# Nico59000/Ternary-image-codec

Measured on AMD Instinct MI355X. Metric: Mpix/s encode+decode 8K RS(26,20), higher is better.
Workload: dtype u8

## Files before the change

ternary-image-codec_amd/csrc/t3_api_decode.cpp:

```cpp
#include <hip/hip_runtime.h>
#include <math.h>
#include <stdio.h>
#include <string.h>

#include <stdlib.h>

#include <algorithm>
#include <mutex>
#include <vector>

#include "../../include/t3hip.h"
#include "t3_ctx.hpp"
#include "t3_dec_plan.hpp"
#include "t3_decode.h"
#include "t3_host.hpp"
#include "t3_repair.h"
#include "t3_window.h"

using namespace t3;

namespace {
struct HdrCheck { HdrExpect ex; uint32_t hs; uint32_t* verdict; const uint8_t* in; };

int launch_hdr_compare(const HdrCheck* h, hipStream_t s) {
    if (!h) return T3_OK;
    hipLaunchKernelGGL(hdr_compare_kernel, dim3(1), dim3(128), 0, s, h->in, h->ex, h->hs, h->verdict);
    HIPCHK(hipGetLastError());
    return T3_OK;
}
template <class A> int settle_header(A& a, const HdrCheck* h, bool whole_frame, hipStream_t s) {
    static const bool no_fold = getenv("T3HIP_HDR_KERNEL") != nullptr;
    if (!h || !a.tile_ctr || !whole_frame || no_fold || h->hs > 96u || ((uintptr_t)h->in & 3u) != 0) return launch_hdr_compare(h, s);
    a.verdict = h->verdict; a.hdr_in = h->in; a.hdr_n = h->hs; memcpy(a.hx, h->ex.b, 96);
    a.fail = a.tile_ctr + 64u * a.n_classes + 16u;
    return T3_OK;
}


int ensure_fx_tables(DecodeTables& tab, int k) {
    const int ki = k_index(k);
    if (!tab.synd_lut[ki]) {
        std::vector<uint32_t> img; build_syndrome_lut(k, img);
        HIPCHK(hipMalloc((void**)&tab.synd_lut[ki], img.size() * 4u));
        HIPCHK(hipMemcpy(tab.synd_lut[ki], img.data(), img.size() * 4u, hipMemcpyHostToDevice));
    }
    if (!tab.roots[ki]) {
        const Field& F = field(); const int t = (26 - k) / 2;
        size_t n = 1; for (int i = 0; i < t; ++i) n *= 27;
        std::vector<uint32_t> tbl(n);
        for (size_t idx = 0; idx < n; ++idx) {
            uint8_t sg[5] = {1, 0, 0, 0, 0}; { size_t v = idx; for (int q = 1; q <= t; ++q) { sg[q] = (uint8_t)(v % 27); v /= 27; } }
            uint32_t mask = 0;
            for (int i = 0; i < 26; ++i) {
                const uint8_t x = F.t.exp[i == 0 ? 0 : 26 - i];
                uint8_t acc = sg[t];
                for (int q = t - 1; q >= 0; --q) acc = F.t.add[F.t.mul[acc * 27 + x] * 27 + sg[q]];
                if (acc == 0) mask |= 1u << i;
            }
            tbl[idx] = mask;
        }
        HIPCHK(hipMalloc((void**)&tab.roots[ki], n * 4));
        HIPCHK(hipMemcpy(tab.roots[ki], tbl.data(), n * 4, hipMemcpyHostToDevice));
    }
    if (!tab.synd_afrag[ki]) {
        std::vector<uint32_t> af; build_mfma_syndrome(k, af);
        HIPCHK(hipMalloc((void**)&tab.synd_afrag[ki], af.size() * 4)); HIPCHK(hipMemcpy(tab.synd_afrag[ki], af.data(), af.size() * 4, hipMemcpyHostToDevice));
    }
    if (!tab.synd_T) {
        std::vector<uint32_t> img; build_syndrome_T(img);
        HIPCHK(hipMalloc((void**)&tab.synd_T, img.size() * 4)); HIPCHK(hipMemcpy(tab.synd_T, img.data(), img.size() * 4, hipMemcpyHostToDevice));
        build_syndrome_T(img, 16);
        HIPCHK(hipMalloc((void**)&tab.synd_T16, img.size() * 4)); HIPCHK(hipMemcpy(tab.synd_T16, img.data(), img.size() * 4, hipMemcpyHostToDevice));
        uint8_t sm[kFx2SmallBytes + kFx2ModBytes]; build_fx2_small(sm); build_fx2_mod(sm + kFx2SmallBytes);
        HIPCHK(hipMalloc((void**)&tab.fx2_small, sizeof sm)); HIPCHK(hipMemcpy(tab.fx2_small, sm, sizeof sm, hipMemcpyHostToDevice));
    }
    if (!tab.fma) {
        const Field& F = field();
        std::vector<uint8_t> t(kFmaBytes, 0);
        for (int x = 0; x < 27; ++x) for (int y = 0; y < 27; ++y) for (int c = 0; c < 27; ++c) t[(size_t)(x * 27 + y) * 27 + c] = F.t.add[c * 27 + F.t.mul[x * 27 + y]];
        HIPCHK(hipMalloc((void**)&tab.fma, t.size())); HIPCHK(hipMemcpy(tab.fma, t.data(), t.size(), hipMemcpyHostToDevice));
    }
    return T3_OK;
}

int rgb_dequant_tables(Ctx& c, const uint8_t** out) {
    uint8_t*& d = c.rgb.dequant;
    if (!d) {
        uint8_t t[328]; memset(t, 0, sizeof t);
        auto cl = [](long v) { return v < 0 ? 0 : (v > 255 ? 255 : v); };
        for (int q = 0; q <= 242; ++q) t[q] = (uint8_t)cl(lround(q * (255.0 / 242.0)));
        for (int q = -40; q <= 40; ++q) t[244 + q + 40] = (uint8_t)cl(lround(128 + q * (128.0 / 40.0)));
        HIPCHK(hipMalloc((void**)&d, sizeof t)); HIPCHK(hipMemcpy(d, t, sizeof t, hipMemcpyHostToDevice));
    }
    *out = d; return T3_OK;
}

template <class A, class F> int bind_groups(Ctx& c, A& a, F attach) {
    std::lock_guard<std::mutex> lk(c.tab_mu);
    for (uint32_t g = 0; g < a.n_grp; ++g) { const int k = 26 - (int)a.grp[g].r; const int rc = ensure_fx_tables(c.dec, k); if (rc) return rc; attach(a.grp[g], k_index(k)); }
    a.fma = c.dec.fma; return T3_OK;
}
int bind_uep(UepPlan& p, void* d_out, uint32_t* d_fail) {
    Ctx& c = ctx(); DecUepArgs& a = p.a;
    { const int rc = bind_groups(c, a, [&](DecUepArgs::Grp& G, int ki) { G.afrag = c.dec.synd_afrag[ki]; G.roots = c.dec.roots[ki]; a.ttab = c.dec.synd_T16; a.small = c.dec.fx2_small; }); if (rc) return rc; }
    a.out = d_out; a.fail = d_fail;
    p.fn = by_r(p.ra, [&](auto A) { return by_r(p.rb, [&](auto B) -> const void* {
        if constexpr (decltype(A)::value >= decltype(B)::value) return (const void*)decode_uep_px_kernel<decltype(A)::value, decltype(B)::value>; else return nullptr; }); });
    if (!p.fn) return T3_E_ARG;
    return resident_grid(c, p.fn, 512, a.lds_bytes, a.n_tiles, true, &p.grid);
}
int bind_stream(StreamPlan& p, void* d_out, uint32_t* d_fail) {
    Ctx& c = ctx(); DecStArgs& a = p.a;
    { const int rc = bind_groups(c, a, [&](DecStArgs::Grp& G, int ki) { G.lut = c.dec.synd_lut[ki]; G.roots = c.dec.roots[ki]; a.tab = c.dec.fxtab; }); if (rc) return rc; }
    a.fail = d_fail; p.e.out = d_out;
    p.emit_fn = p.to_pixels ? (const void*)emit_stream_kernel<true> : (const void*)emit_stream_kernel<false>;
    { const int rc = resident_grid(c, (const void*)decode_stream_kernel, 512, a.lds_bytes, a.n_tiles, false, &p.grid); if (rc) return rc; }
    return resident_grid(c, p.emit_fn, 512, p.e.lds_bytes, p.e.n_steps, false, &p.emit_grid);
}

int launch_fixed_fused(FusedPlan& p, const uint8_t* body, const HdrCheck* hdr, hipStream_t s) {
    Ctx& c = ctx(); DecFx2Args& a = p.a; const uint32_t grid = p.grid;
    a.in = body;
#ifdef T3_DEC_STAMPS
    static uint64_t* d_dbg = nullptr; static int calls = 0;
    if (!d_dbg) HIPCHK(hipMalloc((void**)&d_dbg, 16 * 8 * 4096));
    HIPCHK(hipMemsetAsync(d_dbg, 0, 16 * 8 * 4096, s));
    a.dbg = d_dbg;
#endif
    if (p.tickets) tile_tickets(c, s, 1, grid, &a.tile_ctr, &a.n_classes);
    { const int rc = settle_header(a, hdr, p.whole_frame, s); if (rc) return rc; }
    void* args[] = {(void*)&a};
    HIPCHK(hipLaunchKernel(p.fn, dim3(grid), dim3(p.threads), args, a.lds_bytes, s));
#ifdef T3_DEC_STAMPS
    if (++calls == 8 && p.tickets) {
        std::vector<uint64_t> h(16 * grid);
        HIPCHK(hipStreamSynchronize(s));
        HIPCHK(hipMemcpy(h.data(), d_dbg, h.size() * 8, hipMemcpyDeviceToHost));
        double acc[16] = {0};
        for (uint32_t w = 0; w < grid; ++w) for (int i = 0; i < 16; ++i) acc[i] += (double)h[16 * w + i];
        fprintf(stderr, "[t3 dec stamps] grid=%u (%d per CU) tiles=%u lds=%u  mean cycles/WG: producer sets+e1=%.0f barrier=%.0f total=%.0f | consumer bm=%.0f rendezvous=%.0f d5=%.0f barrier=%.0f total=%.0f  clock=%.3f GHz  us/WG=%.1f\n",
                grid, (int)((grid + c.n_cu - 1) / c.n_cu), a.n_tiles, a.lds_bytes, acc[0] / grid, acc[1] / grid, acc[6] / grid, acc[8 + 2] / grid, acc[8 + 3] / grid, acc[8 + 4] / grid, acc[8 + 5] / grid, acc[8 + 6] / grid,
                acc[6] / acc[7] * 0.1, acc[7] / grid * 0.01);
        uint64_t s0 = ~0ull, s1 = 0, e1 = 0; int late = 0;
        for (uint32_t w = 0; w < grid; ++w) { s0 = std::min(s0, h[16 * w + 2]); s1 = std::max(s1, h[16 * w + 2]); e1 = std::max(e1, h[16 * w + 3]); }
        for (uint32_t w = 0; w < grid; ++w) if (h[16 * w + 2] - s0 > 1000) ++late;
        fprintf(stderr, "[t3 dec stamps]   prologue (kernel entry -> first tile's input landed, wave 0): mean %.0f cycles/WG\n", acc[4] / grid);
        fprintf(stderr, "[t3 dec stamps]   timeline (us from first loop start): last start=%.1f last end=%.1f  workgroups starting >10 us late=%d\n", (s1 - s0) * 0.01, (e1 - s0) * 0.01, late);
    }
#endif
    return T3_OK;
}

int launch_fixed_uep(UepPlan& p, const uint8_t* body, const HdrCheck* hdr, hipStream_t s) {
    Ctx& c = ctx(); DecUepArgs& a = p.a;
    void* d_e; int rc = scratch(c, Scratch::StreamWork, (size_t)a.n_sym + 64, &d_e, s); if (rc) return rc;
    a.in = body; a.edge = (uint8_t*)d_e;
    tile_tickets(c, s, 2, p.grid, &a.tile_ctr, &a.n_classes);
    rc = settle_header(a, hdr, true, s); if (rc) return rc;
    void* args[] = {(void*)&a};
    HIPCHK(hipLaunchKernel(p.fn, dim3(p.grid), dim3(512), args, a.lds_bytes, s));
    HIPCHK(hipLaunchKernel((const void*)uep_edge_kernel, dim3((3u * a.n_tiles + 1u + 255u) / 256u), dim3(256), args, 0, s));
    return T3_OK;
}

int launch_fixed_stream(StreamPlan& p, const uint8_t* body, const HdrCheck* hdr, hipStream_t s) {
    void* d_y; int rc = scratch(ctx(), Scratch::StreamWork, (size_t)p.a.n_sym + 64, &d_y, s); if (rc) return rc;
    p.a.in = body; p.a.ystream = (uint8_t*)d_y; p.e.ystream = (const uint8_t*)d_y;
    rc = launch_hdr_compare(hdr, s); if (rc) return rc;
    void* args[] = {(void*)&p.a}; void* eargs[] = {(void*)&p.e};
    HIPCHK(hipLaunchKernel((const void*)decode_stream_kernel, dim3(p.grid), dim3(512), args, p.a.lds_bytes, s));
    HIPCHK(hipLaunchKernel(p.emit_fn, dim3(p.emit_grid), dim3(512), eargs, p.e.lds_bytes, s));
    return T3_OK;
}

int decode_body(const void* d_in, uint64_t n_in, const t3_cfg& cfg, uint64_t n_raw, const uint8_t next[3],
                void* d_out, uint64_t cap_units, uint64_t* n_out, int to_pixels, uint32_t* d_fail, hipStream_t s, const HdrCheck* hdr) {
    const bool fixed = cfg.mode == T3_MODE_FIXED;
    const bool want_rgb = to_pixels == 2;
    if (((uintptr_t)d_in & 1u) != 0 || (to_pixels == 1 && ((uintptr_t)d_out & 1u) != 0)) return T3_E_ARG;
    if (want_rgb && !fixed) return 1;
    Ctx& c = ctx();
    DecArgs a; memset(&a, 0, sizeof a);
    EmitArgs e; memset(&e, 0, sizeof e);
    a.in = (const uint8_t*)d_in; a.fail = d_fail; a.tab = c.d_tab; a.fixed = fixed ? 1 : 0;
    const ScrCycle sc = scrambler_cycle_from_next(next, cfg.seed_s0);
    a.cyc24 = sc.cyc24; a.pre0 = sc.pre[0]; a.pre1 = sc.pre[1];
    a.beacon_on = (cfg.beacon_enabled && cfg.beacon_words_period > 0) ? 1 : 0; a.period = cfg.beacon_words_period; a.slot = cfg.beacon_band_slot;
    uint64_t use_syms, n_words, total = 0;
    if (!fixed) {
        DecLayoutCompat D; plan_decode_compat(n_in, cfg, D);
        a.hdr_syms = 54;
        for (int b = 0; b < 9; ++b) { a.band_k[b] = D.band_k[b]; a.band_blocks[b] = D.band_blocks[b]; a.band_first[b] = total; a.band_off[b] = D.use_off[b]; total += D.band_blocks[b]; }
        use_syms = D.use_syms; n_words = D.out_words;
    } else {
        t3_layout L; int rc = plan(n_raw, cfg, L); if (rc) return T3_E_HEADER;
        if (L.out_words > n_in) return T3_E_HEADER;
        a.hdr_syms = 90; a.n_sym = L.n_sym;
        for (int b = 0; b < 9; ++b) { a.band_k[b] = L.band_k[b]; a.band_blocks[b] = L.band_blocks[b]; a.band_first[b] = total; a.band_off[b] = L.band_body_off[b]; total += L.band_blocks[b]; }
        use_syms = L.n_sym; n_words = n_raw;
        const uint64_t funits = want_rgb ? cap_units : to_pixels ? 2 * n_words : n_words;
        if (want_rgb && (cap_units > 2 * n_words || cap_units + 1 < 2 * n_words || L.interleave2d)) return 1;
        if (want_rgb && !single_k(L)) return 1;
        if (funits <= cap_units && (!to_pixels || ((uintptr_t)d_out & 15u) == 0) && !generic_decode() && 9 * n_in < (1ull << 32)) {
            const bool bcn_ok = L.beacon_on && cfg.beacon_band_slot < 9 && cfg.beacon_words_period >= 2 && cfg.beacon_words_period < (1u << 27) && getenv("T3HIP_BEACON_PASS") == nullptr;
            const uint64_t bytes = L.beacon_on ? L.body_syms : 9 * n_in; const uint32_t hs = L.beacon_on ? 0u : L.header_syms;
            FusedPlan fp; UepPlan up; StreamPlan sp;
            const FusedForm form = (FusedForm)to_pixels;
            int path = 0, frc = bcn_ok ? plan_fixed_fused(9 * n_in, L.header_syms, L, sc, funits, form, fp, cfg.beacon_band_slot, cfg.beacon_words_period)
                                       : plan_fixed_fused(bytes, hs, L, sc, funits, form, fp);
            if (frc == 1 && want_rgb) return 1;
            if (frc == 1 && to_pixels == 1) { path = 1; frc = plan_fixed_uep(bytes, hs, cfg, L, sc, funits, getenv("T3HIP_TWO_KERNEL_DECODE") != nullptr, up); }
            static const uint32_t lut_bytes[4] = {synd_lut_bytes(24), synd_lut_bytes(22), synd_lut_bytes(20), synd_lut_bytes(18)};
            if (frc == 1) { path = 2; frc = plan_fixed_stream(bytes, hs, cfg, L, sc, funits, to_pixels, lut_bytes, sp); }
            if (frc == T3_OK) frc = path == 0 ? bind_fused(fp, d_out, d_fail) : path == 1 ? bind_uep(up, d_out, d_fail) : bind_stream(sp, d_out, d_fail);
            if (frc < 0) return frc;
            if (frc == T3_OK) {
                const uint8_t* body = (const uint8_t*)d_in;
                if (L.beacon_on && !(path == 0 && bcn_ok)) {
                    void* d_b; int brc = scratch(c, Scratch::StreamBody, L.body_syms + 64, &d_b, s); if (brc) return brc;
                    DebeaconArgs d; d.framed = (const uint8_t*)d_in + L.header_syms; d.framed_bytes = 9 * n_in - L.header_syms; d.body = (uint8_t*)d_b; d.body_syms = L.body_syms; d.period = cfg.beacon_words_period; d.slot = cfg.beacon_band_slot;
                    if (L.body_syms) { hipLaunchKernelGGL(debeacon_kernel, dim3(blocks_for((L.body_syms + 15) / 16, 1u << 20)), dim3(256), 0, s, d); HIPCHK(hipGetLastError()); }
                    body = (const uint8_t*)d_b;
                }
                frc = path == 0 ? launch_fixed_fused(fp, body, hdr, s) : path == 1 ? launch_fixed_uep(up, body, hdr, s) : launch_fixed_stream(sp, body, hdr, s);
                if (frc == T3_OK) *n_out = funits;
                return frc;
            }
        }
    }
    if (want_rgb) return 1;
    a.total_blocks = total;
    const uint64_t units = to_pixels ? 2 * n_words : n_words;
    *n_out = units;
    if (units > cap_units) return T3_E_CAPACITY;
    void* d_use; int rc = scratch(c, Scratch::StreamWork, use_syms + 64, &d_use, s); if (rc) return rc;
    rc = launch_hdr_compare(hdr, s); if (rc) return rc;
    a.use = (uint8_t*)d_use;
    if (total) { hipLaunchKernelGGL(dec_gather_rs_kernel, dim3(blocks_for(total, 1u << 20)), dim3(256), 0, s, a); HIPCHK(hipGetLastError()); }
    e.use = (const uint8_t*)d_use; e.use_syms = use_syms; e.out = d_out; e.n_words = n_words; e.to_pixels = to_pixels ? 1 : 0;
    const bool il = cfg.profile == T3_P5_RS26_22_2D && cfg.tile_w && cfg.tile_h && use_syms;
    e.il_on = il ? 1 : 0;
    if (il) fill_interleave(e, cfg, use_syms);
    if (n_words) { hipLaunchKernelGGL(dec_emit_kernel, dim3(blocks_for(n_words, 1u << 20)), dim3(256), 0, s, e); HIPCHK(hipGetLastError()); }
    return T3_OK;
}

int read_header(const void* d_in, uint64_t n_in, int mode, t3_cfg* seen, uint64_t* n_raw, uint8_t next[3], hipStream_t s) {
    const uint64_t hw = mode == T3_MODE_FIXED ? 10 : 6;
    if (n_in < hw) return T3_E_HEADER;
    Ctx& c = ctx();
    std::lock_guard<std::mutex> lk(c.mail_mu);
    uint8_t*& h = c.mail.header;
    if (!h) HIPCHK(hipHostMalloc((void**)&h, 128, hipHostMallocDefault));
    HIPCHK(hipMemcpyAsync(h, d_in, hw * 9, hipMemcpyDeviceToHost, s));
    HIPCHK(hipStreamSynchronize(s));
    uint8_t hb[96]; memcpy(hb, h, hw * 9);
    return header_parse(hb, n_in, mode, *seen, n_raw, next);
}

int fill_window_crop(WinCropArgs& a, const void* d_run, uint64_t first_px, uint64_t stream_px, uint32_t fw, uint32_t fh, uint32_t x0, uint32_t y0, uint32_t w, uint32_t h,
                     void* d_out, bool rgb) {
    Ctx& c = ctx();
    memset(&a, 0, sizeof a);
    if (rgb) { std::lock_guard<std::mutex> lk(c.tab_mu); const int rc = rgb_dequant_tables(c, &a.dq); if (rc) return rc; }
    a.run = (const uint8_t*)d_run; a.out = (uint8_t*)d_out; a.first_px = first_px; a.stream_px = stream_px;
    a.out_bytes = (uint64_t)w * h * (rgb ? 3u : 6u);
    a.lead = (uint32_t)((uintptr_t)d_out & 15u); a.n_gran = (a.lead + a.out_bytes + 15u) / 16u;
    a.fw = fw; a.fh = fh; a.x0 = x0; a.y0 = y0; a.w = w; a.h = h;
    a.wide = a.out_bytes >= (1ull << 31) ? 1u : 0u;
    if (!a.wide) a.div_row = to_dev(fastdiv(rgb ? w : 3u * w)); else a.div_row.d = rgb ? w : 3u * w;
    return a.n_gran > (1ull << 38) || 3ull * w >= (1ull << 32) ? T3_E_ARG : T3_OK;
}
int launch_window_crop(const void* d_run, uint64_t first_px, uint64_t stream_px, uint32_t fw, uint32_t fh, uint32_t x0, uint32_t y0, uint32_t w, uint32_t h,
                       void* d_out, int out_fmt, hipStream_t s) {
    WinCropArgs a; const bool rgb = out_fmt == 2;
    { const int rc = fill_window_crop(a, d_run, first_px, stream_px, fw, fh, x0, y0, w, h, d_out, rgb); if (rc) return rc; }
    const void* fn = rgb ? (const void*)window_crop_kernel<true> : (const void*)window_crop_kernel<false>;
    void* args[] = {(void*)&a};
    HIPCHK(hipLaunchKernel(fn, dim3((unsigned)((a.n_gran + 255u) / 256u)), dim3(256), args, 0, s));
    return T3_OK;
}
int launch_window_crop_frames(const void* d_run, uint64_t run_stride, uint64_t first_px, uint64_t stream_px, uint32_t fw, uint32_t fh, uint32_t x0, uint32_t y0,
                              uint32_t w, uint32_t h, void* d_out, uint64_t out_stride, int out_fmt, uint32_t n_frames, hipStream_t s) {
    WinCropFramesArgs fa; memset(&fa, 0, sizeof fa);
    const bool rgb = out_fmt == 2;
    { const int rc = fill_window_crop(fa.a, d_run, first_px, stream_px, fw, fh, x0, y0, w, h, d_out, rgb); if (rc) return rc; }
    fa.run_stride = run_stride; fa.out_stride = out_stride;
    if (n_frames > 65535u || (((uintptr_t)d_run | (uintptr_t)d_out | run_stride | out_stride) & 15u)) return T3_E_ARG;
    const void* fn = rgb ? (const void*)window_crop_frames_kernel<true> : (const void*)window_crop_frames_kernel<false>;
    void* args[] = {(void*)&fa};
    HIPCHK(hipLaunchKernel(fn, dim3((unsigned)((fa.a.n_gran + 255u) / 256u), n_frames), dim3(256), args, 0, s));
    return T3_OK;
}
// ... 415 lines not shown
```

ternary-image-codec_amd/csrc/t3_decode.h:

```cpp
#pragma once
#include <stdint.h>

#include "t3_device.h"
#include "t3_rs_core.h"

namespace t3 {

struct DecArgs {
    const uint8_t* in;
    uint8_t* use;
    uint32_t* fail;
    const RsTables* tab;
    uint32_t fixed;
    uint32_t hdr_syms;
    uint32_t band_k[9];
    uint64_t band_blocks[9];
    uint64_t band_first[9];
    uint64_t band_off[9];
    uint64_t total_blocks;
    uint64_t n_sym;
    uint32_t beacon_on, period, slot;
    uint32_t cyc24, pre0, pre1;
};

struct EmitArgs {
    const uint8_t* use; uint64_t use_syms;
    void* out; uint64_t n_words;
    uint32_t to_pixels;
    uint32_t il_on, il_w, il_A; DevDiv div_A, div_w;
};

struct FxTables {
    uint8_t mul[729], add[729], sub[729];
    uint8_t inv[27], neg[27], exp[26];
    uint8_t descr[3][32];
    uint8_t pad_[37];
};
static_assert(sizeof(FxTables) == 2400, "FxTables layout");
constexpr int kFxHdr = 512, kFxTab = kFxHdr, kFxLut = 3072;

constexpr int kFx2Cnt = 160, kFx2Sync = 168, kFx2Abort = 172, kFx2Next = 176, kFx2FailWg = 184, kFx2Small = 192;
#ifndef T3_DEC_PX_THREADS
#define T3_DEC_PX_THREADS 512
#endif
#ifndef T3_DEC_PX_AREG
#define T3_DEC_PX_AREG 2
#endif
#ifndef T3_DEC_PX_TCOP
#define T3_DEC_PX_TCOP 16
#endif
#ifndef T3_DEC_PX_NB
#define T3_DEC_PX_NB 52
#endif
#ifndef T3_DEC_QCAP
#define T3_DEC_QCAP 256
#endif
constexpr int kFx2ModSeq = 3072, kFx2TSeq = 3584, kFx2ModPx = 512, kFx2TPx = 1024, kFx2QCap = T3_DEC_QCAP;
constexpr uint32_t kEraQCap = 512;
static_assert(T3_DEC_PX_THREADS % 128 == 0 && T3_DEC_PX_THREADS <= 1024 && T3_DEC_PX_NB % 26 == 0 && 9 * T3_DEC_PX_NB <= T3_DEC_PX_THREADS && T3_DEC_PX_NB < 2048, "pixel-decoder geometry");
struct DecFx2Args {
    const uint8_t* in; uint64_t in_bytes;
    void* out; uint64_t n_units;
    uint32_t* fail;
    const uint32_t* ttab; const uint8_t* small; const uint32_t* afrag;
    const uint8_t* fma; uint32_t fma_off;
    const uint32_t* roots;
    uint32_t k, nb, n_tiles, TS;
    DevDiv div_nb;
    uint32_t n_sym;
    uint32_t hdr_syms;
    uint32_t band_blocks[9]; uint64_t band_body_off[9]; uint32_t band_boff6[9];
    uint32_t cyc24, pre0, pre1;
    uint32_t* tile_ctr; uint32_t n_classes;
    uint32_t* verdict; const uint8_t* hdr_in; uint32_t hdr_n; uint32_t hx[24];
    uint32_t pat[48], pat_off;
    uint32_t y_off, y_stride, q_off, q_stride, o_off, af_off, lds_bytes;
    uint32_t bcn_slot, bcn_pb; DevDiv bcn_div;
    const uint8_t* dq; uint32_t dq_off;
    uint64_t* dbg;
};

struct DecFramesArgs {
    DecFx2Args a;
    uint64_t in_stride, out_stride;
    uint32_t n_frames, n_total;
    DevDiv div_tiles;
};

struct DecEraWinArgs {
    DecFx2Args a;
    uint32_t fw; DevDiv div_fw;
    uint32_t x0, y0, w, rows_end;
    uint32_t first_px, n_px;
};
struct DecEraWinFramesArgs { DecEraWinArgs w; uint64_t in_stride, out_stride; uint32_t n_frames, n_total; DevDiv div_tiles; };

constexpr int kUepMaxGrp = 2;
struct DecUepArgs {
    const uint8_t* in; uint64_t in_bytes;
    void* out; uint64_t n_units;
    uint32_t* fail;
    const uint32_t* ttab; const uint8_t* small; const uint8_t* fma; uint32_t fma_off;
    struct Grp { uint32_t r, nb, n_items, af_off, q_rel, q_cap; DevDiv div_nb; const uint32_t* afrag; const uint32_t* roots; uint8_t bands[12]; } grp[kUepMaxGrp];
    uint32_t n_grp;
    uint32_t pair_tab[8];
    uint32_t TS, n_tiles, n_sym, hdr_syms;
    uint32_t band_blocks[9]; uint64_t band_body_off[9]; uint32_t band_boff6[9];
    uint32_t pat[48], pat_off, rec_off;
    uint32_t y_off, y_stride, q_off, q_stride, lds_bytes;
    uint32_t* tile_ctr; uint32_t n_classes;
    uint32_t* verdict; const uint8_t* hdr_in; uint32_t hdr_n; uint32_t hx[24];
    uint32_t il_on, il_w, il_A; DevDiv div_A, div_w;
    uint8_t* edge;
};

constexpr int kStMaxGrp = 4;
struct DecStArgs {
    const uint8_t* in; uint64_t in_bytes;
    uint8_t* ystream;
    uint32_t* fail;
    const FxTables* tab; const uint8_t* fma; uint32_t fma_off;
    struct Grp { uint32_t r, nb, n_items, wave0, n_waves, lut_off, lut_bytes; const uint32_t* lut; const uint32_t* roots; uint8_t bands[12]; } grp[kStMaxGrp];
    uint32_t n_grp, n_slots;
    uint32_t n_tiles, TS;
    uint32_t n_sym, hdr_syms;
    uint32_t band_blocks[9]; uint64_t band_body_off[9]; uint32_t band_boff6[9];
    uint32_t cyc24, pre0, pre1;
    uint32_t y_off, lds_bytes;
};
struct EmitStArgs {
    const uint8_t* ystream; uint32_t n_sym;
    void* out; uint64_t n_units;
    uint32_t span;
    uint32_t n_steps;
    uint32_t il_on, il_w, il_A, il_fast;
    DevDiv div_A, div_w;
    uint32_t sym_off, o_off, lds_bytes;
};
struct DescrArgs { uint8_t* words; uint64_t n_bytes; uint32_t cyc24, pre0, pre1; };
constexpr int kStageBlocks = 64, kStageThreads = 9 * 64, kStageRunBytes = 9 * 26 * kStageBlocks;
struct StageDecArgs {
    const uint8_t* body;
    uint8_t* out;
    uint64_t* n_valid;
    const RsTables* tab;
    uint32_t band_k[9], band_fixed[9];
    uint64_t band_off[9];
    uint64_t nb;
    uint32_t bcn_band;
    uint64_t bcn_blocks;
    DevDiv div_p1;
};
struct HdrExpect { uint8_t b[96]; };
struct DebeaconArgs { const uint8_t* framed; uint64_t framed_bytes; uint8_t* body; uint64_t body_syms; uint32_t period, slot; };

#if defined(__HIPCC__)
__global__ void dec_gather_rs_kernel(const DecArgs a);
template <int R, bool BCN> __global__ void decode_fixed_kernel(const DecFx2Args a);
template <int R, bool RGB, bool BCN> __global__ void decode_fixed_px_kernel(const DecFx2Args a);
template <int R, bool RGB, bool BCN> __global__ void decode_era_px_kernel(const DecFx2Args a);
__global__ void era_verdict_kernel(const uint32_t* rep6, uint32_t* verdict4);
template <int R, bool RGB, bool BCN> __global__ void decode_era_frames_px(const DecFramesArgs fa);
template <int R, bool RGB, bool BCN> __global__ void decode_era_window_px(const DecEraWinArgs wa);
template <int R, bool RGB, bool BCN> __global__ void decode_era_frames_window_px(const DecEraWinFramesArgs fa);
template <int R, bool RGB, bool BCN = false> __global__ void dec_frames_px(const DecFramesArgs fa);
__global__ void decode_stream_kernel(const DecStArgs a);
template <int RA, int RB> __global__ void decode_uep_px_kernel(const DecUepArgs a);
__global__ void uep_edge_kernel(const DecUepArgs a);
template <bool TO_PIXELS> __global__ void emit_stream_kernel(const EmitStArgs a);
__global__ void debeacon_kernel(const DebeaconArgs a);
__global__ void dec_emit_kernel(const EmitArgs a);
__global__ void descramble_words_kernel(const DescrArgs a);
__global__ void stage_decode_kernel(const StageDecArgs a);
__global__ void fill_u64_kernel(uint64_t* p, uint64_t v);
__global__ void rs_decode_blocks_kernel(uint8_t* code, uint64_t n_blocks, int k, int fixed, const RsTables* tab, uint8_t* data, uint8_t* ok);
__global__ void inject_errors_kernel(uint8_t* syms, uint64_t n_blocks, uint32_t seed, int max_err);
__global__ void hdr_compare_kernel(const uint8_t* in, HdrExpect expect, uint32_t n, uint32_t* mismatch);
#endif

}
```

ternary-image-codec_amd/csrc/t3_decode_px_body.inc:

```
    constexpr uint32_t TCOP = T3_DEC_PX_TCOP, TBASE = kFx2TPx, MT = kFx2ModPx, QCAP = kFx2QCap;
    constexpr uint32_t NW = T3_DEC_PX_THREADS / 128;
    const uint32_t tid = threadIdx.x, lane = tid & 63u, wave = __builtin_amdgcn_readfirstlane(tid >> 6);
#ifdef T3_DEC_STAMPS
    const uint64_t st_entry = __builtin_amdgcn_s_memtime(); uint64_t st_first = 0;
#endif
    const Tickets tk = tickets_setup(a);
    tk.first(tid);
    uint32_t* const failp = a.verdict ? (uint32_t*)(lds + kFx2FailWg) : a.fail;
    if (tid == 0) *(uint32_t*)(lds + kFx2FailWg) = 0u;
    stage_constants<TCOP, TBASE, MT>(a, tid, blockDim.x);
    if constexpr (RGB) { if (tid < 82u) *(uint32_t*)(lds + a.dq_off + 4u * tid) = ((const uint32_t*)a.dq)[tid]; }
    __syncthreads();
#ifdef T3_DEC_STAMPS
    uint64_t st_acc[6] = {0, 0, 0, 0, 0, 0}, st_prev = __builtin_amdgcn_s_memtime(), st_t0 = st_prev, st_rt0 = __builtin_amdgcn_s_memrealtime();
#endif
    if (a.verdict && px_header_wg(args) && wave == 2u * NW - 1u) {
        uint32_t want = 0;
#pragma unroll
        for (uint32_t q = 0; q < 24; ++q) want = lane == q ? a.hx[q] : want;
        px_header_check(args, want, lane);
    }
    const uint8_t* body = a.in + a.hdr_syms;
    const uint32_t n_items = 9u * a.nb;
    const uint32_t units_tile = (a.TS / 13u) * 3u;
    uint32_t cur = blockIdx.x, nxt = tk.next(1u);

    if (wave < NW) {
        const uint32_t n = lane & 31u, h = lane >> 5;
        Geo geo[2][2]; uint32_t off0[2][2];
        const uint32_t t_off = 26u * a.nb;
#pragma unroll
        for (uint32_t p = 0; p < 2; ++p) for (uint32_t q = 0; q < 2; ++q) geo[p][q] = fx2_geo<R>(wave * 128u + p * 64u + q * 32u + n, n_items, a.nb, a.div_nb, 0u, off0[p][q]);
        auto has = [&](uint32_t pass, uint32_t set, uint32_t tile) -> bool { Geo g = geo[pass][set]; asm volatile("" : "+v"(g)); return fx2_has_block<R>(g, tile, a.n_tiles, a.nb); };
        auto run_of = [&](uint32_t pass, uint32_t set, uint32_t tile, const uint8_t* fbody) -> Run<BCN> { return load_run<BCN>(a, fbody, has(pass, set, tile) ? off0[pass][set] + tile * t_off + 10u * h : 0u); };
        constexpr uint32_t AREG = BCN ? 0u : T3_DEC_PX_AREG;
        v4i Ak[AREG ? AREG : 1u];
#pragma unroll
        for (uint32_t st = 0; st < AREG; ++st) Ak[st] = *T3_LDS(const v4i, a.af_off + 16u * (64u * st + lane));
        Run<BCN> PA, PB;
        PA.w = u32x4{0, 0, 0, 0}; PB.w = PA.w; if constexpr (BCN) { PA.x = 16u << 8; PB.x = PA.x; PA.w4 = 0; PB.w4 = 0; }
        if (cur < px_n_tiles(args)) { PA = run_of(0, 0, px_tile(args, cur), px_body(args, body, cur)); PB = run_of(0, 1, px_tile(args, cur), px_body(args, body, cur)); }
        for (uint32_t k = 0; cur < px_n_tiles(args); ++k) {
            const uint32_t tile = px_tile(args, cur), buf = k & 1u;
            const uint32_t y_off = a.y_off + buf * a.y_stride, q_off = a.q_off + buf * a.q_stride;
            const uint32_t u2 = 2u * mod3_u32(tile * a.nb), toff = tile * t_off;
            uint32_t raw; asm volatile("" : "=v"(raw));
#pragma unroll
            for (uint32_t pass = 0; pass < 2; ++pass) {
                uint32_t LA[4], LB[4];
                run_bytes<BCN>(PA, LA); run_bytes<BCN>(PB, LB);
#ifdef T3_DEC_STAMPS
                if (k == 0u && pass == 0u) { asm volatile("s_waitcnt vmcnt(0)" ::: "memory"); st_first = __builtin_amdgcn_s_memtime() - st_entry; }
#endif
                if (pass == 1u) {
                    asm volatile("" : "+v"(LA[0]), "+v"(LA[1]), "+v"(LA[2]), "+v"(LA[3]), "+v"(LB[0]), "+v"(LB[1]), "+v"(LB[2]), "+v"(LB[3]));
                    if (tid == 0u && tk.dyn) raw = tk.request();
                }
                {
                    const uint32_t np = pass ^ 1u, nt = pass == 0 ? cur : nxt;
                    if (nt < px_n_tiles(args)) { PA = run_of(np, 0, px_tile(args, nt), px_body(args, body, nt)); PB = run_of(np, 1, px_tile(args, nt), px_body(args, body, nt)); }
                }
                if (wave * 128u + pass * 64u < n_items) {
                    Geo gA = geo[pass][0], gB = geo[pass][1]; asm volatile("" : "+v"(gA), "+v"(gB));
                    const Blk bA = fx2_block(gA, off0[pass][0] + toff, fx2_has_block<R>(gA, tile, a.n_tiles, a.nb), u2, y_off);
                    const Blk bB = fx2_block(gB, off0[pass][1] + toff, fx2_has_block<R>(gB, tile, a.n_tiles, a.nb), u2, y_off);
                    const Synd sA = fx2_set<R, TCOP, TBASE, MT, 0, R, AREG>(bA, LA, lane, a.af_off, a.pat_off, Ak);
                    Synd sB; sB.lo = 0; sB.hi = 0;
                    if (wave * 128u + pass * 64u + 32u < n_items) sB = fx2_set<R, TCOP, TBASE, MT, 0, R, AREG>(bB, LB, lane, a.af_off, a.pat_off, Ak);
                    fx2_own_blocks<R>(a.roots, a.fma_off, px_fail(args, failp, cur), sA, sB, bA, bB, (h ? gB : gA) & 0xFFFFu, lane, kFx2Cnt + 4u * buf, q_off, QCAP);
                }
            }
            if (tid == 0u) tk.publish(buf, raw, nxt);
            T3D_STAMP(0);
            barrier_lds();
            T3D_STAMP(1);
            cur = nxt; nxt = tk.next(buf);
        }
        barrier_lds();
    } else {
        const uint32_t cw = wave - NW;
        uint32_t prev = 0;
        for (uint32_t k = 0;; ++k) {
            if (k >= 1u) {
                const uint32_t tile = px_tile(args, prev), buf = (k - 1u) & 1u;
                const uint32_t y_off = a.y_off + buf * a.y_stride, q_off = a.q_off + buf * a.q_stride;
                const uint32_t Q = min(*(const uint32_t*)(lds + kFx2Cnt + 4u * buf), QCAP);
                for (uint32_t e0 = cw * 64u; e0 < Q; e0 += 64u * NW) {
                    const uint32_t e = e0 + lane;
                    if (e < Q) {
                        if constexpr (R == 6 && !BCN) fx3_queue_entry(a.roots, a.fma_off, px_fail(args, failp, prev), e, q_off, QCAP, y_off);
                        else fx2_queue_entry<R>(a.roots, a.fma_off, px_fail(args, failp, prev), e, q_off, QCAP, y_off);
                    }
                }
                T3D_STAMP(2);
                consumer_rendezvous<NW>(k, px_fail(args, failp, prev), lane);
                if (tid == 64u * NW) *(uint32_t*)(lds + kFx2Cnt + 4u * buf) = 0;
                T3D_STAMP(3);
                const uint64_t unit0 = (uint64_t)tile * units_tile;
                const uint32_t n_here = (uint32_t)min((uint64_t)units_tile, a.n_units > unit0 ? a.n_units - unit0 : 0ull);
                for (uint32_t j = cw * 64u + lane; 4u * j < a.TS / 13u; j += 64u * NW) fx2_pixels12<RGB>(a, j, y_off, unit0, n_here, px_out_off(args, prev));
                T3D_STAMP(4);
            }
            barrier_lds();
            T3D_STAMP(5);
            if (cur >= px_n_tiles(args)) break;
            prev = cur; cur = nxt; nxt = tk.next(k & 1u);
        }
    }
    px_finish(tk, args, tid);
#ifdef T3_DEC_STAMPS
    if ((tid == 0 || tid == 64u * NW) && a.dbg) {
        uint64_t* d = a.dbg + 16ull * blockIdx.x + (tid ? 8 : 0);
        for (int i = 0; i < 6; ++i) d[i] = st_acc[i];
        d[6] = __builtin_amdgcn_s_memtime() - st_t0; d[7] = __builtin_amdgcn_s_memrealtime() - st_rt0;
        if (tid == 0) { d[2] = st_rt0; d[3] = __builtin_amdgcn_s_memrealtime(); d[4] = st_first; }
    }
#endif
```

ternary-image-codec_amd/csrc/t3_decode_wg.h:

```cpp
#pragma once
#include "t3_decode_fx.h"
#include "t3_host.hpp"

namespace t3 {
namespace {

template <class A>
__device__ __forceinline__ void stage_band_rows(const A& a) {
#pragma unroll
    for (int b = 0; b < 9; ++b) { Row r; r.blocks = a.band_blocks[b]; r.boff6 = a.band_boff6[b]; r.body_off = a.band_body_off[b]; *(Row*)(lds + 16 * b) = r; }
}

template <uint32_t TCOP, uint32_t TBASE, uint32_t MT, class A>
__device__ __forceinline__ void stage_fx2_tables(const A& a, const uint32_t* const& afrag, const uint32_t& af_off, const uint32_t tid, const uint32_t nthr) {
    for (uint32_t i = tid * 16u; i < (uint32_t)kFx2SmallBytes; i += nthr * 16u) *(uint4*)(lds + kFx2Small + i) = *(const uint4*)(a.small + i);
    for (uint32_t i = tid * 16u; i < (uint32_t)kFx2ModBytes; i += nthr * 16u) *(uint4*)(lds + MT + i) = *(const uint4*)(a.small + kFx2SmallBytes + i);
    for (uint32_t i = tid * 16u; i < 3u * 27u * 4u * TCOP; i += nthr * 16u) *(uint4*)(lds + TBASE + i) = *(const uint4*)((const uint8_t*)a.ttab + i);
    for (uint32_t i = tid * 16u; i < 19696u; i += nthr * 16u) *(uint4*)(lds + a.fma_off + i) = *(const uint4*)(a.fma + i);
    for (uint32_t i = tid * 16u; i < 3072u; i += nthr * 16u) *(uint4*)(lds + af_off + i) = *(const uint4*)((const uint8_t*)afrag + i);
}
template <class A>
__device__ __forceinline__ void stage_pattern_rows(const A& a, const uint32_t tid) {
    if (tid == 64u) {
#pragma unroll
        for (int i = 0; i < 48; ++i) *(uint32_t*)(lds + a.pat_off + 4 * i) = a.pat[i];
    }
}

struct Tickets {
    bool dyn; uint32_t grid, NC, cls, wgc; uint32_t* ctr;
    __device__ __forceinline__ void first(const uint32_t tid) const { if (tid == 0) *(uint32_t*)(lds + kFx2Next + 4u) = dyn ? cls + NC * (wgc + atomicAdd(ctr, 1u)) : blockIdx.x + grid; }
    __device__ __forceinline__ uint32_t request() const { return atomicAdd(ctr, 1u); }
    __device__ __forceinline__ void publish(const uint32_t buf, const uint32_t& raw, const uint32_t& nxt) const {
        *(uint32_t*)(lds + kFx2Next + 4u * buf) = dyn ? cls + NC * (wgc + raw) : nxt + grid;
    }
    __device__ __forceinline__ uint32_t next(const uint32_t buf) const { return __builtin_amdgcn_readfirstlane(*(const uint32_t*)(lds + kFx2Next + 4u * buf)); }
    template <class A>
    __device__ __forceinline__ void finish(const A& a, const uint32_t tid) const {
        if (dyn && tid == 0u) {
            if (a.verdict) { const uint32_t wgf = *(const uint32_t*)(lds + kFx2FailWg); if (wgf) atomicAdd(a.fail, wgf); }
            asm volatile("s_waitcnt vmcnt(0)" ::: "memory");
            if (atomicAdd(a.tile_ctr + 64u * NC, 1u) == grid - 1u) {
                if (a.verdict) a.verdict[1] = atomicExch(a.fail, 0u);
                for (uint32_t c = 0; c <= NC; ++c) __hip_atomic_store(a.tile_ctr + 64u * c, 0u, __ATOMIC_RELAXED, __HIP_MEMORY_SCOPE_AGENT);
            }
        }
    }
};
template <class A>
__device__ __forceinline__ Tickets tickets_setup(const A& a) {
    Tickets t;
    t.grid = gridDim.x; t.dyn = a.tile_ctr != nullptr;
    t.NC = t.dyn ? a.n_classes : 1u; t.cls = blockIdx.x % t.NC;
    t.wgc = (t.grid - t.cls + t.NC - 1u) / t.NC;
    t.ctr = a.tile_ctr + 64u * t.cls;
    return t;
}

template <class A>
__device__ __forceinline__ void header_check_wave(const A& a, const uint32_t want, const uint32_t lane) {
    bool mis = false;
    if (4u * lane < a.hdr_n) {
        const uint32_t nb = min(4u, a.hdr_n - 4u * lane), mask = nb >= 4u ? 0xFFFFFFFFu : (1u << (8u * nb)) - 1u;
        mis = ((((const uint32_t*)a.hdr_in)[lane] ^ want) & mask) != 0u;
    }
    const bool any = __builtin_amdgcn_ballot_w64(mis) != 0;
    if (lane == 0) a.verdict[0] = any ? 1u : 0u;
}

template <uint32_t NW>
__device__ __forceinline__ void consumer_rendezvous(const uint32_t target, uint32_t* const failp, const uint32_t lane) {
    asm volatile("s_waitcnt lgkmcnt(0)" ::: "memory");
    uint32_t* const sync = (uint32_t*)__builtin_assume_aligned(lds + kFx2Sync, 4);
    if (lane == 0) __hip_atomic_fetch_add(sync, 1u, __ATOMIC_RELAXED, __HIP_MEMORY_SCOPE_WORKGROUP);
    uint32_t spins = 0;
    while (__hip_atomic_load(sync, __ATOMIC_RELAXED, __HIP_MEMORY_SCOPE_WORKGROUP) < NW * target) {
        __builtin_amdgcn_s_sleep(1);
        if (++spins > (1u << 22)) { if (lane == 0) { *(uint32_t*)(lds + kFx2Abort) = 1u; atomicAdd(failp, 1u << 20); } break; }
    }
}

__device__ __forceinline__ void store_px12(uint8_t* const g, const uint32_t (&o)[18], const uint32_t p0, const uint32_t n_px) {
    if (p0 + 12u <= n_px) {
#pragma unroll
        for (int d = 0; d < 4; ++d) { U128a<8> w; w.v = u32x4{o[4 * d], o[4 * d + 1], o[4 * d + 2], o[4 * d + 3]}; *(U128a<8>*)(g + 16 * d) = w; }
        U64a<8> w2; w2.v = u32x2{o[16], o[17]}; *(U64a<8>*)(g + 64) = w2;
    } else {
#pragma unroll
        for (uint32_t hh = 0; hh < 36; ++hh)
            if (p0 + hh / 3u < n_px) *(uint16_t*)(g + 2u * hh) = (uint16_t)(o[hh >> 1] >> (16u * (hh & 1u)));
    }
}

}
}
```

Before: 126,200.

## Replace per-tile workgroup barriers with LDS counter handoff between producer and consumer waves

In the R=6 non-beacon pixel decoder, the full workgroup barrier between producer (syndrome/BM) waves and consumer (pixel emit) waves is replaced by LDS counters. These track ready tiles, freed double buffers and a small ring of published tile IDs. Producers and consumers can then drift up to one tile apart instead of lock-stepping at every barrier, which hides per-tile imbalance. The cost is spin-wait polling with s_sleep and more complex ordering, which relies on lgkmcnt drains, and there is a risk of subtle races or extra LDS traffic.

After: 122,600. 0.971x the previous value.

```diff
diff --git a/ternary-image-codec_amd/csrc/t3_api_decode.cpp b/ternary-image-codec_amd/csrc/t3_api_decode.cpp
--- a/ternary-image-codec_amd/csrc/t3_api_decode.cpp
+++ b/ternary-image-codec_amd/csrc/t3_api_decode.cpp
@@ -138,7 +138,7 @@
         HIPCHK(hipMemcpy(h.data(), d_dbg, h.size() * 8, hipMemcpyDeviceToHost));
         double acc[16] = {0};
         for (uint32_t w = 0; w < grid; ++w) for (int i = 0; i < 16; ++i) acc[i] += (double)h[16 * w + i];
-        fprintf(stderr, "[t3 dec stamps] grid=%u (%d per CU) tiles=%u lds=%u  mean cycles/WG: producer sets+e1=%.0f barrier=%.0f total=%.0f | consumer bm=%.0f rendezvous=%.0f d5=%.0f barrier=%.0f total=%.0f  clock=%.3f GHz  us/WG=%.1f\n",
+        fprintf(stderr, "[t3 dec stamps] grid=%u (%d per CU) tiles=%u lds=%u  mean cycles/WG: producer sets+e1=%.0f wait=%.0f total=%.0f | consumer bm=%.0f rendezvous=%.0f d5=%.0f wait=%.0f total=%.0f  clock=%.3f GHz  us/WG=%.1f\n",
                 grid, (int)((grid + c.n_cu - 1) / c.n_cu), a.n_tiles, a.lds_bytes, acc[0] / grid, acc[1] / grid, acc[6] / grid, acc[8 + 2] / grid, acc[8 + 3] / grid, acc[8 + 4] / grid, acc[8 + 5] / grid, acc[8 + 6] / grid,
                 acc[6] / acc[7] * 0.1, acc[7] / grid * 0.01);
         uint64_t s0 = ~0ull, s1 = 0, e1 = 0; int late = 0;
diff --git a/ternary-image-codec_amd/csrc/t3_decode.h b/ternary-image-codec_amd/csrc/t3_decode.h
--- a/ternary-image-codec_amd/csrc/t3_decode.h
+++ b/ternary-image-codec_amd/csrc/t3_decode.h
@@ -40,11 +40,18 @@
 constexpr int kFxHdr = 512, kFxTab = kFxHdr, kFxLut = 3072;
 
 constexpr int kFx2Cnt = 160, kFx2Sync = 168, kFx2Abort = 172, kFx2Next = 176, kFx2FailWg = 184, kFx2Small = 192;
+constexpr int kFx2Handoff = 352;
 #ifndef T3_DEC_PX_THREADS
 #define T3_DEC_PX_THREADS 512
 #endif
 #ifndef T3_DEC_PX_AREG
 #define T3_DEC_PX_AREG 2
+#endif
+#ifndef T3_DEC_PX_HANDOFF
+#define T3_DEC_PX_HANDOFF 1
+#endif
+#ifndef T3_DEC_PX_HO_SLEEP
+#define T3_DEC_PX_HO_SLEEP 1
 #endif
 #ifndef T3_DEC_PX_TCOP
 #define T3_DEC_PX_TCOP 16
diff --git a/ternary-image-codec_amd/csrc/t3_decode_px_body.inc b/ternary-image-codec_amd/csrc/t3_decode_px_body.inc
--- a/ternary-image-codec_amd/csrc/t3_decode_px_body.inc
+++ b/ternary-image-codec_amd/csrc/t3_decode_px_body.inc
@@ -1,11 +1,13 @@
     constexpr uint32_t TCOP = T3_DEC_PX_TCOP, TBASE = kFx2TPx, MT = kFx2ModPx, QCAP = kFx2QCap;
     constexpr uint32_t NW = T3_DEC_PX_THREADS / 128;
+    constexpr bool HO = T3_DEC_PX_HANDOFF != 0 && R == 6 && !BCN;
     const uint32_t tid = threadIdx.x, lane = tid & 63u, wave = __builtin_amdgcn_readfirstlane(tid >> 6);
 #ifdef T3_DEC_STAMPS
     const uint64_t st_entry = __builtin_amdgcn_s_memtime(); uint64_t st_first = 0;
 #endif
     const Tickets tk = tickets_setup(a);
-    tk.first(tid);
+    if constexpr (HO) { if (tid == 0) { HandoffLds h0{nullptr}; ho_start(h0, blockIdx.x, tk.first_id()); } }
+    else tk.first(tid);
     uint32_t* const failp = a.verdict ? (uint32_t*)(lds + kFx2FailWg) : a.fail;
     if (tid == 0) *(uint32_t*)(lds + kFx2FailWg) = 0u;
     stage_constants<TCOP, TBASE, MT>(a, tid, blockDim.x);
@@ -23,7 +25,7 @@
     const uint8_t* body = a.in + a.hdr_syms;
     const uint32_t n_items = 9u * a.nb;
     const uint32_t units_tile = (a.TS / 13u) * 3u;
-    uint32_t cur = blockIdx.x, nxt = tk.next(1u);
+    uint32_t cur = blockIdx.x, nxt = HO ? 0u : tk.next(1u);
 
     if (wave < NW) {
         const uint32_t n = lane & 31u, h = lane >> 5;
@@ -55,10 +57,24 @@
                 if (pass == 1u) {
                     asm volatile("" : "+v"(LA[0]), "+v"(LA[1]), "+v"(LA[2]), "+v"(LA[3]), "+v"(LB[0]), "+v"(LB[1]), "+v"(LB[2]), "+v"(LB[3]));
                     if (tid == 0u && tk.dyn) raw = tk.request();
+                    if constexpr (HO) {
+                        T3D_STAMP(0);
+                        HandoffLds hm{px_fail(args, failp, cur)};
+                        if (!ho_tile_id(hm, k + 1u, nxt)) goto px_loops_done;
+                        T3D_STAMP(1);
+                    }
                 }
                 {
                     const uint32_t np = pass ^ 1u, nt = pass == 0 ? cur : nxt;
                     if (nt < px_n_tiles(args)) { PA = run_of(np, 0, px_tile(args, nt), px_body(args, body, nt)); PB = run_of(np, 1, px_tile(args, nt), px_body(args, body, nt)); }
+                }
+                if constexpr (HO) {
+                    if (pass == 0u) {
+                        T3D_STAMP(0);
+                        HandoffLds hm{px_fail(args, failp, cur)};
+                        if (!ho_acquire_buffer(hm, NW, k)) goto px_loops_done;
+                        T3D_STAMP(1);
+                    }
                 }
                 if (wave * 128u + pass * 64u < n_items) {
                     Geo gA = geo[pass][0], gB = geo[pass][1]; asm volatile("" : "+v"(gA), "+v"(gB));
@@ -70,43 +86,69 @@
                     fx2_own_blocks<R>(a.roots, a.fma_off, px_fail(args, failp, cur), sA, sB, bA, bB, (h ? gB : gA) & 0xFFFFu, lane, kFx2Cnt + 4u * buf, q_off, QCAP);
                 }
             }
-            if (tid == 0u) tk.publish(buf, raw, nxt);
-            T3D_STAMP(0);
-            barrier_lds();
-            T3D_STAMP(1);
-            cur = nxt; nxt = tk.next(buf);
+            if constexpr (HO) {
+                HandoffLds hm{px_fail(args, failp, cur)};
+                ho_release_tile(hm, k);
+                if (tid == 0u) ho_publish_id(hm, k + 2u, tk.drawn_id(raw, nxt));
+                cur = nxt;
+            } else {
+                if (tid == 0u) tk.publish(buf, raw, nxt);
+                T3D_STAMP(0);
+                barrier_lds();
+                T3D_STAMP(1);
+                cur = nxt; nxt = tk.next(buf);
+            }
         }
-        barrier_lds();
+        if constexpr (!HO) barrier_lds();
     } else {
         const uint32_t cw = wave - NW;
+#define T3_PX_CONSUME(KT)                                                                                                                   \
+        {                                                                                                                                    \
+            const uint32_t tile = px_tile(args, prev), buf = (KT) & 1u;                                                                      \
+            const uint32_t y_off = a.y_off + buf * a.y_stride, q_off = a.q_off + buf * a.q_stride;                                           \
+            const uint32_t Q = min(*(const uint32_t*)(lds + kFx2Cnt + 4u * buf), QCAP);                                                      \
+            for (uint32_t e0 = cw * 64u; e0 < Q; e0 += 64u * NW) {                                                                           \
+                const uint32_t e = e0 + lane;                                                                                                \
+                if (e < Q) {                                 \
+                    if constexpr (R == 6 && !BCN) fx3_queue_entry(a.roots, a.fma_off, px_fail(args, failp, prev), e, q_off, QCAP, y_off);    \
+                    else fx2_queue_entry<R>(a.roots, a.fma_off, px_fail(args, failp, prev), e, q_off, QCAP, y_off);                          \
+                }                                                                                                                            \
+            }                                                                                                                                \
+            T3D_STAMP(2);                                                                                                                    \
+            consumer_rendezvous<NW>((KT) + 1u, px_fail(args, failp, prev), lane);    \
+                           \
+            if (tid == 64u * NW) *(uint32_t*)(lds + kFx2Cnt + 4u * buf) = 0;                                                                 \
+            T3D_STAMP(3);                                                                                                                    \
+            const uint64_t unit0 = (uint64_t)tile * units_tile;                                                                              \
+            const uint32_t n_here = (uint32_t)min((uint64_t)units_tile, a.n_units > unit0 ? a.n_units - unit0 : 0ull);                       \
+            for (uint32_t j = cw * 64u + lane; 4u * j < a.TS / 13u; j += 64u * NW) fx2_pixels12<RGB>(a, j, y_off, unit0, n_here, px_out_off(args, prev)); \
+            T3D_STAMP(4);                                                                                                                    \
+        }
         uint32_t prev = 0;
-        for (uint32_t k = 0;; ++k) {
-            if (k >= 1u) {
-                const uint32_t tile = px_tile(args, prev), buf = (k - 1u) & 1u;
-                const uint32_t y_off = a.y_off + buf * a.y_stride, q_off = a.q_off + buf * a.q_stride;
-                const uint32_t Q = min(*(const uint32_t*)(lds + kFx2Cnt + 4u * buf), QCAP);
-                for (uint32_t e0 = cw * 64u; e0 < Q; e0 += 64u * NW) {
-                    const uint32_t e = e0 + lane;
-                    if (e < Q) {
-                        if constexpr (R == 6 && !BCN) fx3_queue_entry(a.roots, a.fma_off, px_fail(args, failp, prev), e, q_off, QCAP, y_off);
-                        else fx2_queue_entry<R>(a.roots, a.fma_off, px_fail(args, failp, prev), e, q_off, QCAP, y_off);
-                    }
-                }
-                T3D_STAMP(2);
-                consumer_rendezvous<NW>(k, px_fail(args, failp, prev), lane);
-                if (tid == 64u * NW) *(uint32_t*)(lds + kFx2Cnt + 4u * buf) = 0;
-                T3D_STAMP(3);
-                const uint64_t unit0 = (uint64_t)tile * units_tile;
-                const uint32_t n_here = (uint32_t)min((uint64_t)units_tile, a.n_units > unit0 ? a.n_units - unit0 : 0ull);
-                for (uint32_t j = cw * 64u + lane; 4u * j < a.TS / 13u; j += 64u * NW) fx2_pixels12<RGB>(a, j, y_off, unit0, n_here, px_out_off(args, prev));
-                T3D_STAMP(4);
+        if constexpr (HO) {
+            for (uint32_t k = 0;; ++k) {
+                HandoffLds hm{px_fail(args, failp, prev)};
+                if (k >= 1u && !ho_tile_id(hm, k, cur)) break;
+                if (cur >= px_n_tiles(args)) break;
+                if (!ho_acquire_tile(hm, NW, k)) break;
+                T3D_STAMP(5);
+                prev = cur;
+                T3_PX_CONSUME(k)
+                ho_release_buffer(hm);
             }
-            barrier_lds();
-            T3D_STAMP(5);
-            if (cur >= px_n_tiles(args)) break;
-            prev = cur; cur = nxt; nxt = tk.next(k & 1u);
+        } else {
+            for (uint32_t k = 0;; ++k) {
+                if (k >= 1u) T3_PX_CONSUME(k - 1u)
+                barrier_lds();
+                T3D_STAMP(5);
+                if (cur >= px_n_tiles(args)) break;
+                prev = cur; cur = nxt; nxt = tk.next(k & 1u);
+            }
         }
+#undef T3_PX_CONSUME
     }
+px_loops_done:
+    if constexpr (HO) barrier_lds();
     px_finish(tk, args, tid);
 #ifdef T3_DEC_STAMPS
     if ((tid == 0 || tid == 64u * NW) && a.dbg) {
diff --git a/ternary-image-codec_amd/csrc/t3_decode_wg.h b/ternary-image-codec_amd/csrc/t3_decode_wg.h
--- a/ternary-image-codec_amd/csrc/t3_decode_wg.h
+++ b/ternary-image-codec_amd/csrc/t3_decode_wg.h
@@ -1,6 +1,8 @@
 #pragma once
 #include "t3_decode_fx.h"
+#include "t3_decode_fx2.h"
 #include "t3_host.hpp"
+#include "t3_tile_handoff.h"
 
 namespace t3 {
 namespace {
@@ -30,6 +32,8 @@
 struct Tickets {
     bool dyn; uint32_t grid, NC, cls, wgc; uint32_t* ctr;
     __device__ __forceinline__ void first(const uint32_t tid) const { if (tid == 0) *(uint32_t*)(lds + kFx2Next + 4u) = dyn ? cls + NC * (wgc + atomicAdd(ctr, 1u)) : blockIdx.x + grid; }
+    __device__ __forceinline__ uint32_t first_id() const { return dyn ? cls + NC * (wgc + atomicAdd(ctr, 1u)) : blockIdx.x + grid; }
+    __device__ __forceinline__ uint32_t drawn_id(const uint32_t& raw, const uint32_t& nxt) const { return dyn ? cls + NC * (wgc + raw) : nxt + grid; }
     __device__ __forceinline__ uint32_t request() const { return atomicAdd(ctr, 1u); }
     __device__ __forceinline__ void publish(const uint32_t buf, const uint32_t& raw, const uint32_t& nxt) const {
         *(uint32_t*)(lds + kFx2Next + 4u * buf) = dyn ? cls + NC * (wgc + raw) : nxt + grid;
@@ -80,6 +84,22 @@
     }
 }
 
+static_assert(kFx2Small + kFx2SmallBytes <= kFx2Handoff && kFx2Handoff + 4 * (int)kHoWords <= (int)kFx2Dummy, "the hand-off words lie between the byte tables and the dummy");
+struct HandoffLds {
+    static constexpr uint32_t kSpinBound = 1u << 22;
+    uint32_t* failp;
+    __device__ __forceinline__ static uint32_t* at(const uint32_t word) { return (uint32_t*)__builtin_assume_aligned(lds + kFx2Handoff + 4u * word, 4); }
+    __device__ __forceinline__ static bool lane0() { return __builtin_amdgcn_mbcnt_hi(~0u, __builtin_amdgcn_mbcnt_lo(~0u, 0u)) == 0u; }
+    __device__ __forceinline__ uint32_t load(const uint32_t word) const { return __builtin_amdgcn_readfirstlane(__hip_atomic_load(at(word), __ATOMIC_RELAXED, __HIP_MEMORY_SCOPE_WORKGROUP)); }
+    __device__ __forceinline__ void add1(const uint32_t word) const { if (lane0()) __hip_atomic_fetch_add(at(word), 1u, __ATOMIC_RELAXED, __HIP_MEMORY_SCOPE_WORKGROUP); }
+    __device__ __forceinline__ void store(const uint32_t word, const uint32_t v) const { __hip_atomic_store(at(word), v, __ATOMIC_RELAXED, __HIP_MEMORY_SCOPE_WORKGROUP); }
+    __device__ __forceinline__ void drain() const { asm volatile("s_waitcnt lgkmcnt(0)" ::: "memory"); }
+    __device__ __forceinline__ void fence() const { asm volatile("" ::: "memory"); }
+    __device__ __forceinline__ void pause() const { __builtin_amdgcn_s_sleep(T3_DEC_PX_HO_SLEEP); }
+    __device__ __forceinline__ bool abort_seen() const { return __builtin_amdgcn_readfirstlane(__hip_atomic_load((uint32_t*)__builtin_assume_aligned(lds + kFx2Abort, 4), __ATOMIC_RELAXED, __HIP_MEMORY_SCOPE_WORKGROUP)) != 0u; }
+    __device__ __forceinline__ void give_up() const { if (lane0()) { *(uint32_t*)(lds + kFx2Abort) = 1u; atomicAdd(failp, 1u << 20); } }
+};
+
 __device__ __forceinline__ void store_px12(uint8_t* const g, const uint32_t (&o)[18], const uint32_t p0, const uint32_t n_px) {
     if (p0 + 12u <= n_px) {
 #pragma unroll
diff --git a/ternary-image-codec_amd/csrc/t3_tile_handoff.h b/ternary-image-codec_amd/csrc/t3_tile_handoff.h
--- /dev/null
+++ b/ternary-image-codec_amd/csrc/t3_tile_handoff.h
@@ -0,0 +1,48 @@
+#pragma once
+#include <stdint.h>
+
+#if defined(__HIPCC__)
+#define T3_HO_FN __host__ __device__ __forceinline__
+#else
+#define T3_HO_FN inline
+#endif
+
+namespace t3 {
+
+enum HandoffWord : uint32_t { kHoReady = 0, kHoFreed = 2, kHoPub = 3, kHoRing = 4 };
+constexpr uint32_t kHoWords = 8, kHoRingSlots = 4, kHoPubStart = 2;
+
+T3_HO_FN constexpr uint32_t ho_ready_word(const uint32_t k) { return (uint32_t)kHoReady + (k & 1u); }
+T3_HO_FN constexpr uint32_t ho_ready_target(const uint32_t nw, const uint32_t k) { return nw * (k / 2u + 1u); }
+T3_HO_FN constexpr uint32_t ho_freed_target(const uint32_t nw, const uint32_t k) { return k < 2u ? 0u : nw * (k - 1u); }
+T3_HO_FN constexpr uint32_t ho_pub_target(const uint32_t j) { return j + 1u; }
+T3_HO_FN constexpr uint32_t ho_ring_word(const uint32_t j) { return (uint32_t)kHoRing + (j & (kHoRingSlots - 1u)); }
+
+template <class M>
+T3_HO_FN bool ho_wait(M& m, const uint32_t word, const uint32_t target) {
+    uint32_t spins = 0;
+#pragma unroll 1
+    while (m.load(word) < target) {
+        if ((++spins & 15u) == 0u && m.abort_seen()) return false;
+        if (spins > M::kSpinBound) { m.give_up(); return false; }
+        m.pause();
+    }
+    m.fence();
+    return true;
+}
+
+template <class M> T3_HO_FN bool ho_acquire_buffer(M& m, const uint32_t nw, const uint32_t k) { return k < 2u || ho_wait(m, kHoFreed, ho_freed_target(nw, k)); }
+template <class M> T3_HO_FN void ho_release_tile(M& m, const uint32_t k) { m.drain(); m.add1(ho_ready_word(k)); }
+template <class M> T3_HO_FN bool ho_acquire_tile(M& m, const uint32_t nw, const uint32_t k) { return ho_wait(m, ho_ready_word(k), ho_ready_target(nw, k)); }
+template <class M> T3_HO_FN void ho_release_buffer(M& m) { m.drain(); m.add1(kHoFreed); }
+template <class M> T3_HO_FN void ho_start(M& m, const uint32_t id0, const uint32_t id1) {
+    m.store(ho_ready_word(0u), 0u); m.store(ho_ready_word(1u), 0u); m.store(kHoFreed, 0u); m.store(ho_ring_word(0u), id0); m.store(ho_ring_word(1u), id1); m.store(kHoPub, kHoPubStart);
+}
+template <class M> T3_HO_FN void ho_publish_id(M& m, const uint32_t j, const uint32_t id) { m.store(ho_ring_word(j), id); m.store(kHoPub, ho_pub_target(j)); }
+template <class M> T3_HO_FN bool ho_tile_id(M& m, const uint32_t j, uint32_t& id) {
+    if (!ho_wait(m, kHoPub, ho_pub_target(j))) return false;
+    id = m.load(ho_ring_word(j));
+    return true;
+}
+
+}
```
